# natir/br

Hardware: AMD Instinct MI355X
Metric: corrected Gbases/sec at k=19, 10 kb ONT-error reads (higher is better)
Workload: dtype u64 k-mers / 1-bit set

## Files before the change

br_amd/csrc/brx_partbuild.hip:

```cpp
#include "brx_internal.hpp"
#include "brx_index.hpp"

#include <stdlib.h>
#include <string.h>
#include <atomic>

namespace brx {
uint64_t scan_tmp_bytes(uint32_t n);
int exclusive_scan_lens(const uint32_t *d_lens, uint32_t n, uint64_t *d_tmp, uint64_t *d_out_offsets,
                        unsigned long long *d_total, hipStream_t s);
}

using namespace brx;

namespace {

constexpr int F_BITS = 12;
constexpr int MAX_LEVELS = 4;
constexpr int MAX_DIGIT_BITS = 9;
static_assert(MAX_DIGIT_BITS <= 9, "the digit scans of the partition passes are written for at most 512 digits");

struct Plan {
    int k, nbits, nlev;
    int bits[MAX_LEVELS];
// ... 825 lines not shown
                incl += u;
        }
        __syncthreads();
        if ((threadIdx.x & 63) == 63)
            wsum[threadIdx.x >> 6] = incl;
        __syncthreads();
        uint64_t base = poff[p];
        for (uint32_t w = 0; w < (threadIdx.x >> 6); w++)
            base += wsum[w];
        uint64_t run[2];
        run[0] = base + incl - mine;
        run[1] = run[0] + tot[0];
        for (uint32_t q = 0; q < BPT; q++) {
            const uint32_t b = threadIdx.x * BPT + q;
            if (b < B)
                coff[p * B + b] = run[q];
        }
        for (uint64_t t = 0; t < nt; t++)
            for (uint32_t q = 0; q < BPT; q++) {
                const uint32_t b = threadIdx.x * BPT + q;
                if (b < B) {
                    pos[B * (io + t) + b] = run[q];
                    run[q] += m[B * (io + t) + b];
                }
            }
        if (p == n_parents - 1 && threadIdx.x == 0)
            coff[n_parents * B] = poff[n_parents];
    }
}

template <int KPT, typename OUT>
__global__ __launch_bounds__(256) void ln_scatter_kernel(LnArgs a)
{
    extern __shared__ __attribute__((aligned(16))) uint8_t lds_raw[];
    __shared__ uint32_t sh_wsum[4];
    const uint32_t T = a.tile;
    const uint32_t B = 1u << a.bits;
    uint32_t *stage_key = (uint32_t *)lds_raw;
    uint16_t *stage_dig = (uint16_t *)(lds_raw + (size_t)T * 4);
    unsigned long long *gbase = (unsigned long long *)(lds_raw + (size_t)T * 6);
    uint32_t *cntv = (uint32_t *)(lds_raw + (size_t)T * 6 + (size_t)B * 8);
    uint32_t *lofs = cntv + B;
    uint32_t *lcur = lofs + B;
    const int shift = a.rem_in - a.bits;
    const uint32_t child_mask = (1u << shift) - 1u;
    OUT *out = (OUT *)a.keys_out;
    const unsigned long long n_items = *a.n_items;
    const ItemRange ir = xcd_items(n_items);
    if (ir.first >= ir.end)
        return;
    constexpr uint32_t OWN = ((1u << MAX_DIGIT_BITS) + 255u) / 256u;
    auto load_rows = [&](unsigned long long item, uint32_t(&rc)[OWN], uint64_t(&rp)[OWN]) {
#pragma unroll
        for (uint32_t q = 0; q < OWN; q++) {
            const uint32_t b = threadIdx.x + 256u * q;
            const uint64_t mi = B * item + (b < B ? b : 0u);
            rc[q] = a.matrix[mi];
            rp[q] = a.pos[mi];
        }
    };
    LnItem it = ln_item_get(ln_item_load(a, ir.first));
    uint32_t key[KPT], rc[OWN];
    uint64_t rp[OWN];
    load_rows(ir.first, rc, rp);
    ln_load<KPT>(a, it, key);
    for (unsigned long long item = ir.first; item < ir.end; item += ir.step) {
#pragma unroll
        for (uint32_t q = 0; q < OWN; q++) {
            const uint32_t b = threadIdx.x + 256u * q;
            if (b < B) {
                cntv[b] = rc[q];
                gbase[b] = rp[q];
            }
        }
        const uint32_t cnt = ln_count(it);
        __syncthreads();
        block_scan_bins(B, cntv, lofs, lcur, sh_wsum);
        __syncthreads();
#pragma unroll
        for (int q = 0; q < KPT; q++)
            if ((uint32_t)q < cnt) {
                const uint32_t d = (key[q] >> shift) & (B - 1u);
                const uint32_t slot = atomicAdd(&lcur[d], 1u);
                stage_key[slot] = key[q] & child_mask;
                stage_dig[slot] = (uint16_t)d;
            }
        __syncthreads();
        const uint32_t n_tile = lofs[B - 1] + cntv[B - 1];
        for (uint32_t idx = threadIdx.x; idx < n_tile; idx += 256) {
            const uint32_t d = stage_dig[idx];
            const uint64_t at = gbase[d] + (idx - lofs[d]);
            if (store_ok(at, a.out_cap))
                out[at] = (OUT)stage_key[idx];
        }
        const unsigned long long next = item + ir.step;
        if (next < ir.end) {
            it = ln_item_get(ln_item_load(a, next));
            load_rows(next, rc, rp);
            ln_load<KPT>(a, it, key);
        }
        __syncthreads();
    }
}

constexpr int P3_WAVES = 4;
constexpr uint32_t F_SIZE = 1u << F_BITS;
constexpr uint32_t CNT_WORDS = F_SIZE / 2;
constexpr uint32_t BIT_WORDS = F_SIZE / 32;
constexpr uint32_t CHUNK_MAX = 65000;

constexpr uint32_t STAGE_KEYS = 704;

constexpr uint32_t EMIT_CAP = 256;

template <bool EMIT, bool BITS>
__global__ __launch_bounds__(64 * P3_WAVES) void final_count_kernel(const uint16_t *__restrict__ keys,
                                                                     const uint64_t *__restrict__ off, uint64_t n_buckets,
                                                                     uint32_t abundance, uint32_t *__restrict__ bits,
                                                                     uint64_t *__restrict__ emit_keys, uint64_t emit_cap,
                                                                     unsigned long long *__restrict__ emit_n)
{
    __shared__ uint32_t cnt_all[P3_WAVES][CNT_WORDS];
    __shared__ uint32_t bit_all[P3_WAVES][BIT_WORDS];
    __shared__ __attribute__((aligned(8))) uint16_t stage_all[P3_WAVES][STAGE_KEYS + 8];
    __shared__ uint64_t emit_all[EMIT ? P3_WAVES : 1][EMIT ? EMIT_CAP : 1];
    const int wave = threadIdx.x >> 6, lane = threadIdx.x & 63;
    uint32_t *cnt = cnt_all[wave];
    uint32_t *bmp = bit_all[wave];
    uint16_t *stage = stage_all[wave];
    uint64_t *ebuf = emit_all[EMIT ? wave : 0];
    uint32_t ecount = 0;
    auto emit_flush = [&]() {
        if (ecount) {
            unsigned long long base = 0;
            if (lane == 0)
                base = atomicAdd(emit_n, (unsigned long long)ecount);
            base = __shfl(base, 0);
            asm volatile("" ::: "memory");
            for (uint32_t q = lane; q < ecount; q += 64)
                if (base + q < emit_cap)
                    emit_keys[base + q] = ebuf[q];
            asm volatile("" ::: "memory");
            ecount = 0;
        }
    };
    for (uint32_t w = lane; w < CNT_WORDS; w += 64)
        cnt[w] = 0;
    for (uint32_t w = lane; w < BIT_WORDS; w += 64)
        bmp[w] = 0;
    auto emit_if = [&](bool flag, uint64_t hkey) {
        const uint64_t bal = __ballot(flag);
        if (bal) {
            if (ecount + 64u > EMIT_CAP)
                emit_flush();
            if (flag)
                ebuf[ecount + __builtin_amdgcn_mbcnt_hi((uint32_t)(bal >> 32), __builtin_amdgcn_mbcnt_lo((uint32_t)bal, 0u))] = hkey;
            ecount += (uint32_t)__builtin_popcountll(bal);
        }
    };
    asm volatile("" ::: "memory");

    const uint64_t n_waves = (uint64_t)gridDim.x * P3_WAVES;
    const uint64_t wid = (uint64_t)blockIdx.x * P3_WAVES + wave;
    const uint64_t per = (n_buckets + n_waves - 1) / n_waves;
    const uint64_t b_lo = wid * per;
    const uint64_t b_hi = (b_lo + per < n_buckets) ? b_lo + per : n_buckets;

    uint64_t g0 = b_lo;
    while (g0 < b_hi) {
        int gmax = (int)((b_hi - g0 < 63) ? b_hi - g0 : 63);
        const uint64_t oi = g0 + (uint64_t)lane;
        const uint64_t offv = off[oi <= n_buckets ? oi : n_buckets];
        const uint64_t gs = __shfl(offv, 0);
        const bool fits = lane >= 1 && lane <= gmax && (offv - gs) <= (uint64_t)STAGE_KEYS;
        const uint64_t fm = __ballot(fits) >> 1;
        int gcount = (fm == ~0ull >> 1) ? 63 : __builtin_ctzll(~fm);
        if (gcount > gmax)
            gcount = gmax;
        const bool staged = gcount > 0;
        if (!staged)
            gcount = 1;
        const uint64_t ge = __shfl(offv, gcount);
        const uint64_t base4 = gs & ~3ull;
        if (staged) {
            const uint32_t nquads = (uint32_t)((ge - base4 + 3) / 4);
            const uint2 *src = reinterpret_cast<const uint2 *>(keys + base4);
            uint2 *dstq = reinterpret_cast<uint2 *>(stage);
            for (uint32_t q = lane; q < nquads; q += 64)
                dstq[q] = src[q];
            asm volatile("" ::: "memory");
        }
        const uint32_t off_lo = (uint32_t)offv, off_hi = (uint32_t)(offv >> 32);
        for (int j = 0; j < gcount; j++) {
            const uint64_t s = ((uint64_t)(uint32_t)__builtin_amdgcn_readlane(off_hi, j) << 32) |
                               (uint64_t)(uint32_t)__builtin_amdgcn_readlane(off_lo, j);
            const uint64_t e = ((uint64_t)(uint32_t)__builtin_amdgcn_readlane(off_hi, j + 1) << 32) |
                               (uint64_t)(uint32_t)__builtin_amdgcn_readlane(off_lo, j + 1);
            const uint64_t n = e - s;
            bool any_bit = false;
            if (n == 0) {
            } else if (staged && n <= 64) {
                const bool act = (uint64_t)lane < n;
                const uint32_t key = act ? stage[(uint32_t)(s - base4) + lane] : 0u;
                const uint32_t word = key & (CNT_WORDS - 1u), half = key >> (F_BITS - 1);
                bool hot = false, cross = false;
                if (act) {
                    const uint32_t old = (atomicAdd(&cnt[word], 1u << (16u * half)) >> (16u * half)) & 0xffffu;
                    const uint32_t c = old + 1u;
                    hot = (c > 255u ? 255u : c) > abundance;
                    cross = old == abundance && abundance < 255u;
                    if (BITS && hot)
                        atomicOr(&bmp[key >> 5], 1u << (key & 31u));
                }
                if (BITS)
                    any_bit = __ballot(hot) != 0ull;
                else if (EMIT)
                    emit_if(cross, (g0 + (uint64_t)j) * F_SIZE + (uint64_t)key);
                asm volatile("" ::: "memory");
                if (act)
                    cnt[word] = 0;
            } else {
                any_bit = true;
                uint64_t done = 0;
                while (done < n) {
                    const uint64_t m = (n - done < CHUNK_MAX) ? n - done : CHUNK_MAX;
                    for (uint64_t i = lane; i < m; i += 64) {
                        const uint32_t kk = staged ? (uint32_t)stage[(uint32_t)(s - base4 + done + i)] : (uint32_t)keys[s + done + i];
                        atomicAdd(&cnt[kk & (CNT_WORDS - 1u)], 1u << (16u * (kk >> (F_BITS - 1))));
                    }
                    asm volatile("" ::: "memory");
                    done += m;
                    if (done < n) {
                        for (uint32_t w = lane; w < CNT_WORDS; w += 64) {
                            const uint32_t v = cnt[w];
                            const uint32_t a0 = v & 0xffffu, a1 = v >> 16;
                            cnt[w] = (a0 > 255u ? 255u : a0) | ((a1 > 255u ? 255u : a1) << 16);
                        }
                        asm volatile("" ::: "memory");
                    }
                }
                for (uint32_t w = lane; w < CNT_WORDS; w += 64) {
                    const uint32_t v = cnt[w];
                    const uint32_t c0 = v & 0xffffu, c1 = v >> 16;
                    const bool s0 = (c0 > 255u ? 255u : c0) > abundance, s1 = (c1 > 255u ? 255u : c1) > abundance;
                    if (BITS) {
                        if (s0)
                            atomicOr(&bmp[w >> 5], 1u << (w & 31u));
                        if (s1)
                            atomicOr(&bmp[(w + CNT_WORDS) >> 5], 1u << (w & 31u));
                    } else if (EMIT) {
                        emit_if(s0, (g0 + (uint64_t)j) * F_SIZE + (uint64_t)w);
                        emit_if(s1, (g0 + (uint64_t)j) * F_SIZE + (uint64_t)(w + CNT_WORDS));
                    }
                    if (v)
                        cnt[w] = 0;
                }
            }
            asm volatile("" ::: "memory");
            if (!BITS)
                continue;
            uint32_t *dst = bits + (g0 + (uint64_t)j) * BIT_WORDS;
            uint32_t w0 = 0, w1 = 0;
            if (any_bit) {
                w0 = bmp[2 * lane];
                w1 = bmp[2 * lane + 1];
                bmp[2 * lane] = 0;
                bmp[2 * lane + 1] = 0;
            }
            *reinterpret_cast<uint2 *>(dst + 2 * lane) = make_uint2(w0, w1);
            asm volatile("" ::: "memory");
            if (EMIT && any_bit) {
                uint64_t rem = (uint64_t)w0 | ((uint64_t)w1 << 32);
                const uint64_t hbase = (g0 + (uint64_t)j) * F_SIZE + 64ull * (uint64_t)lane;
                for (;;) {
                    const uint64_t bal = __ballot(rem != 0ull);
                    if (!bal)
                        break;
                    if (ecount + 64u > EMIT_CAP)
                        emit_flush();
                    if (rem) {
                        const uint32_t pos = ecount + __builtin_amdgcn_mbcnt_hi((uint32_t)(bal >> 32),
                                                                                __builtin_amdgcn_mbcnt_lo((uint32_t)bal, 0u));
                        ebuf[pos] = hbase + (uint64_t)__builtin_ctzll(rem);
                        rem &= rem - 1ull;
                    }
                    ecount += (uint32_t)__builtin_popcountll(bal);
                }
            }
        }
        g0 += (uint64_t)gcount;
    }
    if (EMIT)
        emit_flush();
}

#ifndef BRX_HF_FLAT
#define BRX_HF_FLAT 1
#endif
constexpr bool HF_FLAT = BRX_HF_FLAT != 0;
constexpr uint32_t HF_VALID = 0x80000000u;
constexpr int HF_CHUNK = 8;
constexpr uint32_t HF_MAX_TRIES = 192;
__host__ __device__ constexpr uint32_t hf_ebuf(int team) { return team > 64 ? 1024u : 512u; }

template <int TEAM, int BLOCK>
__global__ __launch_bounds__(BLOCK) void hash_final_kernel(const uint32_t *__restrict__ keys, const uint64_t *__restrict__ off,
                                                         uint64_t n_buckets, int R, uint32_t abundance, uint32_t log_t,
                                                         uint64_t *__restrict__ emit_keys, uint64_t emit_cap,
                                                         unsigned long long *__restrict__ emit_n,
                                                         const unsigned long long *__restrict__ dup, uint32_t min_lt, float ratio_forced)
{
    extern __shared__ __attribute__((aligned(16))) uint8_t hf_lds[];
    constexpr int TEAMS = BLOCK / TEAM;
    constexpr uint32_t EB = hf_ebuf(TEAM);
    const uint32_t MIN_LT = min_lt;
    const uint32_t Tmax = 1u << log_t;
    const int team = threadIdx.x / TEAM, tl = threadIdx.x % TEAM;
    uint32_t *tab = (uint32_t *)hf_lds + (size_t)team * Tmax;
    unsigned long long *ebuf = (unsigned long long *)(hf_lds + (size_t)TEAMS * Tmax * 4) + (size_t)team * EB;
    uint32_t *ctl = (uint32_t *)(hf_lds + (size_t)TEAMS * Tmax * 4 + (size_t)TEAMS * EB * 8) + team * 4;
    auto team_sync = [&]() {
        if (TEAM > 64)
            __syncthreads();
        else
            __builtin_amdgcn_fence(__ATOMIC_ACQ_REL, "wavefront");
    };
    auto flush = [&]() {
        team_sync();
        const uint32_t ne = ctl[0] < EB ? ctl[0] : EB;
        __shared__ unsigned long long sh_base[TEAMS];
        if (tl == 0)
            sh_base[team] = ne ? atomicAdd(emit_n, (unsigned long long)ne) : 0ull;
        team_sync();
        const unsigned long long base = sh_base[team];
        for (uint32_t q = tl; q < ne; q += TEAM)
            if (base + q < emit_cap)
                emit_keys[base + q] = ebuf[q];
        team_sync();
        if (tl == 0)
            ctl[0] = 0;
        team_sync();
    };
    if (tl == 0) {
        ctl[0] = 0;
        ctl[1] = 0;
    }
    team_sync();
    float ratio = 1.0f;
    if (dup) {
        const float d = (float)dup[0], t = (float)dup[1];
        if (t > 0.0f)
            ratio = fminf(1.0f, 1.25f * d / t + 0.01f);
    }
    if (ratio_forced > 0.0f)
        ratio = ratio_forced;
    const uint64_t n_teams = (uint64_t)gridDim.x * TEAMS;
    for (uint64_t b = (uint64_t)blockIdx.x * TEAMS + team; b < n_buckets; b += n_teams) {
        const uint64_t s0 = off[b], n = off[b + 1] - s0;
        if (n == 0)
            continue;
        const uint64_t n_eff = (uint64_t)((float)n * ratio) + 1ull;
        uint32_t lp = 0;
        while (lp < (uint32_t)R && (n_eff >> lp) > (uint64_t)(Tmax / 8u * 5u))
            lp++;
        uint32_t lt = log_t;
        if (lp == 0) {
            const uint32_t want = (uint32_t)n_eff * 5u / 2u;
            lt = MIN_LT < log_t ? MIN_LT : log_t;
            while (lt < log_t && (1u << lt) < want)
                lt++;
        }
        uint32_t T = 1u << lt;
        for (uint32_t pass = 0; pass < (1u << lp);) {
            for (uint32_t q = tl * 4u; q < T; q += TEAM * 4u)
                *(uint4 *)(tab + q) = make_uint4(0u, 0u, 0u, 0u);
            team_sync();
            for (uint64_t i0 = 0; i0 < n; i0 += (uint64_t)TEAM * HF_CHUNK) {
              uint32_t kbuf[HF_CHUNK];
#pragma unroll
              for (int c = 0; c < HF_CHUNK; c++) {
                  const uint64_t i = i0 + (uint64_t)c * TEAM + tl;
                  kbuf[c] = i < n ? keys[s0 + i] : 0xffffffffu;
              }
              if constexpr (HF_FLAT && TEAM > 64) {
#pragma unroll
              for (int c = 0; c < HF_CHUNK; c++) {
                const uint32_t key = kbuf[c];
                uint32_t pend = (key != 0xffffffffu && !(lp && (key >> ((uint32_t)R - lp)) != pass)) ? 1u : 0u;
                uint32_t h = (key * 0x9E3779B1u) >> (32u - lt);
                const uint32_t mine = HF_VALID | (key << 11);
                for (uint32_t tries = 0; __any(pend); tries++) {
                    const uint32_t e = tab[h];
                    uint32_t r = e;
                    if (pend & (uint32_t)(e == 0u))
                        r = atomicCAS(&tab[h], 0u, mine | 1u);
                    const uint32_t won = (uint32_t)(e == 0u) & (uint32_t)(r == 0u);
                    const uint32_t same = (uint32_t)((r & 0xfffff800u) == mine);
                    if (pend & same & (uint32_t)((r & 0x400u) == 0u))
                        atomicAdd(&tab[h], 1u);
                    pend &= ~(won | same) & 1u;
                    if (tries >= HF_MAX_TRIES) {
                        if (pend)
                            ctl[1] = 1;
                        pend = 0;
                    }
                    h = (h + 1u) & (T - 1u);
                }
              }
              } else {
#pragma unroll
              for (int c = 0; c < HF_CHUNK; c++) {
                const uint32_t key = kbuf[c];
                if (key == 0xffffffffu || (lp && (key >> ((uint32_t)R - lp)) != pass))
                    continue;
                uint32_t h = (key * 0x9E3779B1u) >> (32u - lt);
                const uint32_t mine = HF_VALID | (key << 11);
                for (uint32_t tries = 0;; tries++) {
                    uint32_t e = tab[h];
                    if (e == 0u) {
                        e = atomicCAS(&tab[h], 0u, mine | 1u);
                        if (e == 0u)
                            break;
                    }
                    if ((e & 0xfffff800u) == mine) {
                        if ((e & 0x7ffu) < 1024u)
                            atomicAdd(&tab[h], 1u);
                        break;
                    }
                    if (tries >= HF_MAX_TRIES) {
                        ctl[1] = 1;
                        break;
                    }
                    h = (h + 1u) & (T - 1u);
                }
              }
              }
            }
            team_sync();
            const uint32_t ovf = ctl[1];
            team_sync();
            if (ovf) {
                if (tl == 0)
                    ctl[1] = 0;
                team_sync();
                if (lt < log_t) {
                    lt = log_t;
                    T = Tmax;
                    continue;
                }
                if (lp + 2u <= (uint32_t)R) {
                    lp += 2u;
                    pass <<= 2;
                    continue;
                }
            }
            for (uint32_t q0 = tl * 4u; q0 < T; q0 += TEAM * 4u) {
                const uint4 e4 = *(const uint4 *)(tab + q0);
                const uint32_t ev[4] = {e4.x, e4.y, e4.z, e4.w};
#pragma unroll
                for (int j = 0; j < 4; j++) {
                    const uint32_t e = ev[j];
                    const uint32_t cnt = e & 0x7ffu;
                    if ((e & HF_VALID) && (cnt > 255u ? 255u : cnt) > abundance) {
                        const unsigned long long hk = (b << R) | (uint64_t)((e >> 11) & 0xfffffu);
                        const uint32_t pos = atomicAdd(&ctl[0], 1u);
                        if (pos < EB) {
                            ebuf[pos] = hk;
                        } else {
                            const unsigned long long gp = atomicAdd(emit_n, 1ull);
                            if (gp < emit_cap)
                                emit_keys[gp] = hk;
                        }
                    }
                }
            }
            team_sync();
            const uint32_t ec = ctl[0];
            team_sync();
            if (ec > EB / 2u)
                flush();
            pass++;
        }
    }
    flush();
}

__global__ __launch_bounds__(1024) void hf_sample_kernel(const uint32_t *__restrict__ keys, const uint64_t *__restrict__ off,
                                                         uint64_t n_buckets, int R, uint32_t log_t, unsigned long long *__restrict__ dup)
{
    extern __shared__ __attribute__((aligned(16))) uint8_t hf_lds[];
    __shared__ uint32_t sh_new;
    uint32_t *tab = (uint32_t *)hf_lds;
    const uint32_t T = 1u << log_t;
    const uint64_t b = (uint64_t)blockIdx.x * n_buckets / gridDim.x;
    const uint64_t s0 = off[b], n = off[b + 1] - s0;
    if (threadIdx.x == 0)
        sh_new = 0;
    uint32_t lp = 0;
    while (lp < (uint32_t)R && (n >> lp) > (uint64_t)(T / 8u * 5u))
        lp++;
    uint32_t fresh = 0;
    for (uint32_t pass = 0; pass < (1u << lp); pass++) {
        __syncthreads();
        for (uint32_t q = threadIdx.x; q < T; q += 1024u)
            tab[q] = 0;
        __syncthreads();
        for (uint64_t i = threadIdx.x; i < n; i += 1024u) {
            const uint32_t key = keys[s0 + i];
            if (lp && (key >> ((uint32_t)R - lp)) != pass)
                continue;
            uint32_t h = (key * 0x9E3779B1u) >> (32u - log_t);
            const uint32_t mine = HF_VALID | (key << 11);
            for (uint32_t tries = 0; tries < T; tries++) {
                uint32_t e = tab[h];
                if (e == 0u) {
                    e = atomicCAS(&tab[h], 0u, mine);
                    if (e == 0u) {
                        fresh++;
                        break;
                    }
                }
                if (e == mine)
                    break;
                h = (h + 1u) & (T - 1u);
            }
        }
    }
    atomicAdd(&sh_new, fresh);
    __syncthreads();
    if (threadIdx.x == 0) {
        atomicAdd(dup, (unsigned long long)sh_new);
        atomicAdd(dup + 1, (unsigned long long)n);
    }
}

constexpr int SP_WAVES = 4;
__global__ __launch_bounds__(64 * SP_WAVES) void final_spectrum_kernel(const uint16_t *__restrict__ keys, const uint64_t *__restrict__ off,
                                                                       uint64_t n_buckets, unsigned long long *__restrict__ hist)
{
    __shared__ uint32_t sp_cnt[SP_WAVES][F_SIZE];
    __shared__ unsigned long long sp_hist[256];
    const int wave = threadIdx.x / 64, lane = threadIdx.x % 64;
    uint32_t *cnt = sp_cnt[wave];
    for (uint32_t q = lane; q < F_SIZE; q += 64)
        cnt[q] = 0;
    for (uint32_t q = threadIdx.x; q < 256; q += 64 * SP_WAVES)
        sp_hist[q] = 0;
    __syncthreads();
    const uint64_t n_waves = (uint64_t)gridDim.x * SP_WAVES;
    for (uint64_t g = (uint64_t)blockIdx.x * SP_WAVES + wave; g < n_buckets; g += n_waves) {
        const uint64_t s0 = off[g], n = off[g + 1] - s0;
        for (uint64_t i = lane; i < n; i += 64)
            atomicAdd(&cnt[keys[s0 + i]], 1u);
        __builtin_amdgcn_fence(__ATOMIC_ACQ_REL, "wavefront");
        for (uint64_t i = lane; i < n; i += 64) {
            const uint32_t c = atomicExch(&cnt[keys[s0 + i]], 0u);
            if (c)
                atomicAdd(&sp_hist[c > 255u ? 255u : c], 1ull);
        }
        __builtin_amdgcn_fence(__ATOMIC_ACQ_REL, "wavefront");
    }
    __syncthreads();
    for (uint32_t q = threadIdx.x; q < 256; q += 64 * SP_WAVES)
        if (sp_hist[q])
            atomicAdd(&hist[q], sp_hist[q]);
}

constexpr int VW_WAVES = 4;
constexpr uint32_t VIEW_PAD = 0xFFFFu;
constexpr uint64_t VW_PER_WAVE = 63ull * 16ull;
__global__ __launch_bounds__(64 * VW_WAVES) void final_view_kernel(uint16_t *keys, const uint64_t *__restrict__ off, uint64_t n_buckets,
                                                                   uint8_t *__restrict__ cnt_out)
{
    __shared__ uint32_t bins_all[VW_WAVES][F_SIZE];
    __shared__ __attribute__((aligned(8))) uint16_t stage_all[VW_WAVES][STAGE_KEYS + 8];
    __shared__ __attribute__((aligned(4))) uint8_t scnt_all[VW_WAVES][STAGE_KEYS + 8];
    __shared__ uint32_t bmp_all[VW_WAVES][BIT_WORDS];
    const int wave = threadIdx.x >> 6, lane = threadIdx.x & 63;
    uint32_t *bins = bins_all[wave];
    uint16_t *stage = stage_all[wave];
    uint8_t *scnt = scnt_all[wave];
    uint32_t *bmp = bmp_all[wave];
    for (uint32_t q = lane; q < F_SIZE; q += 64)
        bins[q] = 0;
    bmp[2 * lane] = 0;
    bmp[2 * lane + 1] = 0;
    asm volatile("" ::: "memory");

    const uint64_t n_chunks = (n_buckets + VW_PER_WAVE * VW_WAVES - 1) / (VW_PER_WAVE * VW_WAVES);
    for (uint64_t chunk = blockIdx.x; chunk < n_chunks; chunk += gridDim.x) {
        const uint64_t b_lo = (chunk * VW_WAVES + (uint64_t)wave) * VW_PER_WAVE;
        const uint64_t b_hi = b_lo + VW_PER_WAVE < n_buckets ? b_lo + VW_PER_WAVE : n_buckets;
        uint64_t g0 = b_lo;
        while (g0 < b_hi) {
            const int gmax = (int)((b_hi - g0 < 63) ? b_hi - g0 : 63);
            const uint64_t oi = g0 + (uint64_t)lane;
            const uint64_t offv = off[oi <= n_buckets ? oi : n_buckets];
            const uint64_t gs = __shfl(offv, 0);
            const bool fits = lane >= 1 && lane <= gmax && (offv - gs) <= (uint64_t)STAGE_KEYS;
            const uint64_t fm = __ballot(fits) >> 1;
            int gcount = (fm == ~0ull >> 1) ? 63 : __builtin_ctzll(~fm);
            if (gcount > gmax)
                gcount = gmax;
            const bool staged = gcount > 0;
            if (!staged)
                gcount = 1;
            const uint64_t ge = __shfl(offv, gcount);
            if (ge == gs) {
                g0 += (uint64_t)gcount;
                continue;
            }
            const uint64_t base4 = gs & ~3ull;
            const uint32_t nquads = (uint32_t)((ge - base4 + 3) / 4);
            if (staged) {
                const uint2 *src = reinterpret_cast<const uint2 *>(keys + base4);
                uint2 *dstq = reinterpret_cast<uint2 *>(stage);
                for (uint32_t q = lane; q < nquads; q += 64)
                    dstq[q] = src[q];
                asm volatile("" ::: "memory");
            }
            const uint32_t off_lo = (uint32_t)offv, off_hi = (uint32_t)(offv >> 32);
            for (int j = 0; j < gcount; j++) {
                const uint64_t s = ((uint64_t)(uint32_t)__builtin_amdgcn_readlane(off_hi, j) << 32) |
                                   (uint64_t)(uint32_t)__builtin_amdgcn_readlane(off_lo, j);
                const uint64_t e = ((uint64_t)(uint32_t)__builtin_amdgcn_readlane(off_hi, j + 1) << 32) |
                                   (uint64_t)(uint32_t)__builtin_amdgcn_readlane(off_lo, j + 1);
                const uint64_t n = e - s;
                if (n == 0)
                    continue;
                const uint32_t sidx = (uint32_t)(s - base4);
                if (staged && n <= 64) {
                    const bool act = (uint64_t)lane < n;
                    const uint32_t key = act ? (uint32_t)stage[sidx + lane] : VIEW_PAD;
                    uint32_t less = 0, mult = 0, distinct = 0;
                    bool lead = false;
                    for (uint64_t rem = __ballot(act); rem; distinct++) {
                        const int i = __builtin_ctzll(rem);
                        const uint32_t ki = (uint32_t)__builtin_amdgcn_readlane((int)key, i);
                        const uint64_t eq = __ballot(act && key == ki);
                        rem &= ~eq;
                        if (ki < key)
                            less++;
                        if (key == ki) {
                            mult = (uint32_t)__builtin_popcountll(eq);
                            lead = lane == i;
                        }
                    }
                    asm volatile("" ::: "memory");
                    if (act && lead) {
                        stage[sidx + less] = (uint16_t)key;
                        scnt[sidx + less] = (uint8_t)(mult > 255u ? 255u : mult);
                    }
                    if (act && (uint32_t)lane >= distinct) {
                        stage[sidx + lane] = (uint16_t)VIEW_PAD;
                        scnt[sidx + lane] = 0;
                    }
                    asm volatile("" ::: "memory");
                    continue;
                }
                for (uint64_t i = lane; i < n; i += 64) {
                    const uint32_t kk = (staged ? (uint32_t)stage[sidx + (uint32_t)i] : (uint32_t)keys[s + i]) & (F_SIZE - 1u);
                    atomicAdd(&bins[kk], 1u);
                    atomicOr(&bmp[kk >> 5], 1u << (kk & 31u));
                }
                __builtin_amdgcn_fence(__ATOMIC_ACQ_REL, "wavefront");
                uint64_t mine = ((uint64_t)bmp[2 * lane + 1] << 32) | (uint64_t)bmp[2 * lane];
                bmp[2 * lane] = 0;
                bmp[2 * lane + 1] = 0;
                const uint32_t nmine = (uint32_t)__builtin_popcountll(mine);
                uint32_t incl = nmine;
                for (int d = 1; d < 64; d <<= 1) {
                    const uint32_t up = (uint32_t)__shfl_up((int)incl, d);
                    if (lane >= d)
                        incl += up;
                }
                const uint32_t pos = (uint32_t)__shfl((int)incl, 63);
                for (uint32_t p = incl - nmine; mine; mine &= mine - 1ull, p++) {
                    const uint32_t h = 64u * (uint32_t)lane + (uint32_t)__builtin_ctzll(mine);
                    const uint32_t v = bins[h];
                    bins[h] = 0;
                    const uint8_t c8 = (uint8_t)(v > 255u ? 255u : v);
                    if (staged) {
                        stage[sidx + p] = (uint16_t)h;
                        scnt[sidx + p] = c8;
                    } else {
                        keys[s + p] = (uint16_t)h;
                        cnt_out[s + p] = c8;
                    }
                }
                for (uint64_t i = (uint64_t)pos + lane; i < n; i += 64) {
                    if (staged) {
                        stage[sidx + (uint32_t)i] = (uint16_t)VIEW_PAD;
                        scnt[sidx + (uint32_t)i] = 0;
                    } else {
                        keys[s + i] = (uint16_t)VIEW_PAD;
                        cnt_out[s + i] = 0;
                    }
                }
                __builtin_amdgcn_fence(__ATOMIC_ACQ_REL, "wavefront");
            }
            if (staged) {
                asm volatile("" ::: "memory");
                for (uint32_t q = lane; q < nquads; q += 64) {
                    const uint64_t at = base4 + 4ull * q;
                    if (at >= gs && at + 4 <= ge) {
                        *reinterpret_cast<uint2 *>(keys + at) = *reinterpret_cast<const uint2 *>(stage + 4u * q);
                        *reinterpret_cast<uint32_t *>(cnt_out + at) = *reinterpret_cast<const uint32_t *>(scnt + 4u * q);
                    } else {
                        for (uint32_t t = 0; t < 4; t++)
                            if (at + t >= gs && at + t < ge) {
                                keys[at + t] = stage[4u * q + t];
                                cnt_out[at + t] = scnt[4u * q + t];
                            }
                    }
                }
                asm volatile("" ::: "memory");
            }
            g0 += (uint64_t)gcount;
        }
    }
}

__global__ __launch_bounds__(256) void merge_segments_kernel(const uint32_t *__restrict__ src,
                                                             const uint64_t *__restrict__ src_off,
                                                             const uint64_t *__restrict__ dst_off,
                                                             const uint64_t *__restrict__ dst_shift, uint32_t B1,
                                                             uint32_t *__restrict__ dst)
{
    for (uint32_t b = blockIdx.x; b < B1; b += gridDim.x) {
        const uint64_t lo = src_off[b], hi = src_off[b + 1];
        const uint64_t base = dst_off[b] + dst_shift[b];
        for (uint64_t i = lo + threadIdx.x; i < hi; i += blockDim.x)
            dst[base + (i - lo)] = src[i];
    }
}

__global__ void add_counts_kernel(const uint64_t *__restrict__ off, uint32_t B1, uint32_t *__restrict__ counts,
                                  uint64_t *__restrict__ shift_out)
{
    const uint32_t b = blockIdx.x * blockDim.x + threadIdx.x;
    if (b < B1) {
        if (shift_out)
            shift_out[b] = counts[b];
        counts[b] += (uint32_t)(off[b + 1] - off[b]);
    }
}

struct PartBatch {
    uint32_t *d_keys = nullptr;
    uint64_t n = 0;
    uint64_t *d_l1off = nullptr;
    DevBuf<uint32_t> own_keys;
    DevBuf<uint64_t> own_l1off;
    bool borrowed() const { return !own_keys; }
    uint64_t cap() const { return own_keys.cap(); }
};

}

namespace brx {

struct PartState {
    Plan pl;
    Plan pl_wide;
    bool use_wide = false;
    std::vector<PartBatch> batches, spare;
// ... 145 lines not shown
    if (st->batches.empty()) {
        *d_keys = nullptr;
        *d_l1off = nullptr;
        *n_keys = 0;
        return BRX_OK;
    }
    if (st->batches.size() != 1 || st->batches[0].borrowed()) {
        set_error("l1_view needs exactly one locally counted batch (have %zu)", st->batches.size());
        return BRX_ERR_ARG;
    }
    *d_keys = st->batches[0].d_keys;
    *d_l1off = st->batches[0].d_l1off;
    *n_keys = st->batches[0].n;
    return BRX_OK;
}

int part_add_partitioned(brx_counter *c, const uint32_t *d_keys, const uint64_t *d_l1off, uint64_t n_keys)
{
    PartState *st = c->part;
    st->view_valid = false;
    if (n_keys == 0)
        return BRX_OK;
    PartBatch b;
    b.d_keys = const_cast<uint32_t *>(d_keys);
    b.d_l1off = const_cast<uint64_t *>(d_l1off);
    b.n = n_keys;
    st->batches.push_back(std::move(b));
    return BRX_OK;
}

static int ensure_matrix(PartState *st, uint64_t n_entries, uint64_t n_pos)
{
    BRX_TRY(ws_reserve(st->d_matrix, (n_entries + 1) * 4));
    BRX_TRY(ws_reserve(st->d_pos, (n_pos + 2) * 8));
    return ws_reserve(st->d_scan_tmp, scan_tmp_bytes((uint32_t)n_entries) + 64);
}

static size_t scatter_lds_bytes(uint32_t tile, int bits)
{
    const size_t B = (size_t)1 << bits;
    return (size_t)tile * 6 + B * 8 + B * 12 + 64;
}

static size_t l1_scatter_lds_bytes(int bits)
{
    const size_t B = (size_t)1 << bits;
    return (size_t)L1_TILE * 4 + B * 8 + B * 12 + 64;
}

int part_add_batch(brx_counter *c, const uint8_t *d_bases, const uint64_t *d_offsets, uint32_t n_reads,
                   uint64_t total_bases, hipStream_t s)
{
    PartState *st = c->part;
    const Plan &pl = st->pl;
    st->view_valid = false;
    if (total_bases == 0 || n_reads == 0)
        return BRX_OK;
    const uint64_t max_keys = total_bases;
    PartBatch b;
    for (size_t i = 0; i < st->spare.size(); i++)
        if (st->spare[i].cap() >= max_keys) {
            b = std::move(st->spare[i]);
            st->spare.erase(st->spare.begin() + (long)i);
            break;
        }
    if (!b.d_keys) {
        BRX_TRY(ws_reserve(b.own_keys, (max_keys + 1) * 4));
        BRX_TRY(b.own_l1off.reserve(pl.nchild[0] + 1, 0, "partition offsets"));
        b.d_keys = b.own_keys;
        b.d_l1off = b.own_l1off;
    }
    const uint32_t B = 1u << pl.bits[0];
    const uint64_t n_items64 = (total_bases + L1_TILE - 1) / L1_TILE;
    if (n_items64 * B >= (1ull << 32)) {
        set_error("batch of %llu bases is too large for one partition pass; split it", (unsigned long long)total_bases);
        return BRX_ERR_UNSUPPORTED;
    }
    const uint32_t n_items = (uint32_t)n_items64;
    const uint64_t n_entries = (uint64_t)B * n_items;
    const char *genv = getenv("BRX_L1_GRID");
    const long gev = genv ? atol(genv) : 0;
    const uint32_t want_ranges = gev > 0 ? (uint32_t)gev : 2560u;
    const uint32_t n_ranges = n_items < want_ranges ? n_items : want_ranges;
    BRX_TRY(ensure_matrix(st, n_entries, ((uint64_t)n_ranges + 1) * B));
    uint64_t *coltot = st->d_pos + (uint64_t)n_ranges * B;
    L1Args a;
    memset(&a, 0, sizeof(a));
    a.bases = d_bases;
    a.offsets = d_offsets;
    a.n_reads = n_reads;
    a.total = total_bases;
    a.n_items = n_items;
    a.k = pl.k;
    a.nbits = pl.nbits;
    a.bits = pl.bits[0];
    a.matrix = st->d_matrix;
    a.n_ranges = n_ranges;
    a.rsum = st->d_pos;
    a.coff = b.d_l1off;
    a.keys_out = b.d_keys;
    a.out_cap = b.cap();
    {
        KernelTimer t("part_l1_hist", s);
        l1_hist_kernel<<<n_ranges, 256, (size_t)B * 4, s>>>(a);
    }
    trace_stage(s, "partition level 1: histograms");
    {
        KernelTimer t("offsets_scan", s);
        col_scan_columns_kernel<<<B, 256, 0, s>>>(st->d_pos, n_ranges, B, coltot);
        col_scan_digits_kernel<<<1, 64, 0, s>>>(coltot, B, b.d_l1off, st->d_scalars + 1);
    }
    {
        KernelTimer t("part_l1_scatter", s);
        const size_t lds1 = l1_scatter_lds_bytes(a.bits);
        if (lds1 > 64 * 1024)
            BRX_HIP(hipFuncSetAttribute((const void *)l1_scatter_kernel, hipFuncAttributeMaxDynamicSharedMemorySize, (int)lds1));
        l1_scatter_kernel<<<n_ranges, 256, lds1, s>>>(a);
    }
    trace_stage(s, "partition level 1: scatter");
    BRX_HIP(hipGetLastError());
    unsigned long long tot = 0;
    BRX_HIP(hipMemcpyAsync(&tot, st->d_scalars + 1, 8, hipMemcpyDeviceToHost, s));
    BRX_HIP(hipStreamSynchronize(s));
    b.n = tot;
    st->batches.push_back(std::move(b));
    return BRX_OK;
}

template <typename OUT>
static int run_level(PartState *st, int l, const uint32_t *keys_in, const uint64_t *poff, uint64_t n_parents, uint64_t total,
                     void *keys_out, hipStream_t s, const char *tag_hist, const char *tag_scatter)
{
    const Plan &pl = st->use_wide ? st->pl_wide : st->pl;
    const uint32_t B = 1u << pl.bits[l];
    static const bool small_tiles = [] { const char *e = getenv("BRX_SMALL_TILES"); return e && *e == '1'; }();
    const uint32_t tile = (pl.bits[l] > 8 || !small_tiles) ? 8192u : 4096u;
    const uint64_t ub_items = total / tile + n_parents + 1;
    const uint64_t n_entries = (uint64_t)B * ub_items;
    if (n_entries >= (1ull << 32)) {
        set_error("partition level %d needs %llu tile counters; split the input into smaller counters", l + 1,
                  (unsigned long long)n_entries);
        return BRX_ERR_UNSUPPORTED;
    }
    {
        BRX_TRY(ws_reserve(st->d_ntiles, (n_parents + 1) * 4));
        BRX_TRY(ws_reserve(st->d_item_off, (n_parents + 2) * 8));
        BRX_TRY(ws_reserve(st->d_items, (ub_items + 1) * sizeof(LnItem)));
    }
    BRX_TRY(ensure_matrix(st, n_entries > n_parents ? n_entries : n_parents, n_entries > n_parents ? n_entries : n_parents));
    tiles_from_offsets_kernel<<<(unsigned)((n_parents + 255) / 256), 256, 0, s>>>(poff, n_parents, tile, st->d_ntiles);
    BRX_TRY(exclusive_scan_lens(st->d_ntiles, (uint32_t)n_parents, st->d_scan_tmp, st->d_item_off, st->d_scalars, s));
    fill_items_kernel<<<(unsigned)((n_parents + 255) / 256), 256, 0, s>>>(poff, st->d_item_off, n_parents, tile, st->d_items);
    trace_stage(s, tag_hist);
    BRX_HIP(hipMemsetAsync(st->d_matrix, 0, n_entries * 4, s));
    LnArgs a;
    memset(&a, 0, sizeof(a));
    a.keys_in = keys_in;
    a.in_cap = total;
    a.items = st->d_items;
    a.n_items = st->d_scalars;
    a.tile = tile;
    a.rem_in = pl.rem_in[l];
    a.bits = pl.bits[l];
    a.matrix = st->d_matrix;
    a.pos = st->d_pos;
    a.keys_out = keys_out;
    a.out_cap = total + 64;
    const int grid = 256 * 8;
    {
        KernelTimer t(tag_hist, s);
        if (tile == 8192u)
            ln_hist_kernel<32><<<grid, 256, (size_t)B * 4, s>>>(a);
        else
            ln_hist_kernel<16><<<grid, 256, (size_t)B * 4, s>>>(a);
    }
    trace_stage(s, "  histograms done");
    {
        KernelTimer t("offsets_scan", s);
        const unsigned g = n_parents < 4096 ? (unsigned)n_parents : 4096u;
        ln_colscan_kernel<<<g, 256, 0, s>>>(st->d_matrix, poff, st->d_item_off, n_parents, B, st->d_pos, st->d_coff[l]);
    }
    {
        KernelTimer t(tag_scatter, s);
        const size_t lds = scatter_lds_bytes(tile, a.bits);
        if (tile == 8192u)
            ln_scatter_kernel<32, OUT><<<grid, 256, lds, s>>>(a);
        else
            ln_scatter_kernel<16, OUT><<<grid, 256, lds, s>>>(a);
    }
    trace_stage(s, tag_scatter);
    BRX_HIP(hipGetLastError());
    return BRX_OK;
}

static int part_finish_impl(brx_counter *c, uint32_t abundance, hipStream_t s, brx_set *dst, unsigned long long *d_hist,
                            bool view = false)
{
    PartState *st = c->part;
    st->view_valid = false;
    const bool no_set = d_hist || view;
    uint64_t total = 0;
    for (auto &b : st->batches)
        total += b.n;
    const char *e_wide = getenv("BRX_WIDE_L2");
    const uint64_t wide_from = e_wide && *e_wide ? strtoull(e_wide, nullptr, 10) : 16384ull;
    const bool lazy_on = [] { const char *e = getenv("BRX_LAZY_BITS"); return !(e && *e == '0'); }();
    st->use_wide = wide_from != 0 && !no_set && dst && (dst->sparse || (index_wanted(c->k) && lazy_on)) &&
                   st->pl_wide.bits[1] != st->pl.bits[1] &&
                   (wide_from == 1 || (st->pl.nlev == 3 ? total / st->pl.nchild[1] > wide_from
                                                        : total / st->pl_wide.nchild[2] > 640));
    const Plan &pl = st->use_wide ? st->pl_wide : st->pl;
    const uint32_t B1 = (uint32_t)pl.nchild[0];

    const uint32_t *keys1 = nullptr;
    const uint64_t *l1off = nullptr;
    if (st->batches.empty() || total == 0) {
        if (view) {
            st->view_empty = true;
            st->view_valid = true;
        }
        if (no_set)
            return BRX_OK;
        if (dst->sparse) {
            BRX_TRY(dst->d_keylist_n.reserve(1, 0, "key list counter"));
            BRX_HIP(hipMemsetAsync(dst->d_keylist_n, 0, 8, s));
            keylist_mark(dst, true);
        } else {
            BRX_HIP(hipMemsetAsync(dst->d_bits, 0, dst->nwords * 4, s));
            dst->bits_stale = false;
        }
        return BRX_OK;
    } else if (st->batches.size() == 1) {
        keys1 = st->batches[0].d_keys;
        l1off = st->batches[0].d_l1off;
    } else {
        BRX_TRY(ws_reserve(st->d_merged, (total + 1) * 4));
        BRX_TRY(ensure_matrix(st, B1 + 1, B1 + 1));
        BRX_HIP(hipMemsetAsync(st->d_cnts, 0, (uint64_t)B1 * 4, s));
        for (auto &b : st->batches)
            add_counts_kernel<<<(B1 + 255) / 256, 256, 0, s>>>(b.d_l1off, B1, st->d_cnts, nullptr);
        BRX_TRY(exclusive_scan_lens(st->d_cnts, B1, st->d_scan_tmp, st->d_l1off_all, st->d_scalars + 1, s));
        BRX_HIP(hipMemsetAsync(st->d_cnts, 0, (uint64_t)B1 * 4, s));
        for (auto &b : st->batches) {
            add_counts_kernel<<<(B1 + 255) / 256, 256, 0, s>>>(b.d_l1off, B1, st->d_cnts, st->d_shift);
            merge_segments_kernel<<<B1 < 4096u ? B1 : 4096u, 256, 0, s>>>(b.d_keys, b.d_l1off, st->d_l1off_all, st->d_shift, B1,
                                                                         st->d_merged);
        }
        keys1 = st->d_merged;
        l1off = st->d_l1off_all;
    }

    BRX_TRY(ws_reserve(st->d_keys_fin, (total + 64) * 2));
    const bool emit = !no_set && (dst->sparse || index_wanted(c->k));
    const bool lazy = emit && !dst->sparse && lazy_on;
    if (emit) {
        const uint64_t div = (dst->sparse || lazy) ? abundance + 1u : (abundance + 1u > 8u ? abundance + 1u : 8u);
        const uint64_t want = total / div + (1ull << 20);
        BRX_TRY(dst->d_keylist.reserve(want, 0, "solid key list"));
        BRX_TRY(dst->d_keylist_n.reserve(1, 0, "key list counter"));
        BRX_HIP(hipMemsetAsync(dst->d_keylist_n, 0, 8, s));
    }
    static const char *hist_tag[MAX_LEVELS] = {"part_l1_hist", "part_l2_hist", "part_l3_hist", "part_l4_hist"};
    static const char *scat_tag[MAX_LEVELS] = {"part_l1_scatter", "part_l2_scatter", "part_l3_scatter", "part_l4_scatter"};
    if (pl.nlev >= 3)
        BRX_TRY(ws_reserve(st->d_keys_mid, (total + 64) * 4));
    if (pl.nlev >= 4)
        BRX_TRY(ws_reserve(st->d_keys_mid2, (total + 64) * 4));
    const uint32_t *kin = keys1;
    const uint64_t *poff = l1off;
    const bool hf_on = [] { const char *e = getenv("BRX_HASH_FINAL"); return !(e && *e == '0'); }();
    const int R_hf = pl.rem_in[pl.nlev - 1];
    const uint64_t nb_hf = pl.nlev >= 2 ? pl.nchild[pl.nlev - 2] : 0;
    static const uint64_t hf_max_avg = [] { const char *e = getenv("BRX_HASH_FINAL_MAX"); return e && *e ? strtoull(e, nullptr, 10) : 131072ull; }();
    const bool hash_final = !no_set && hf_on && (dst->sparse || lazy) && pl.nlev >= 3 && R_hf <= 20 && total / nb_hf <= hf_max_avg;
    for (int l = 1; l < pl.nlev; l++) {
        if (hash_final && l == pl.nlev - 1)
            break;
        if (l == pl.nlev - 1) {
            BRX_TRY(run_level<uint16_t>(st, l, kin, poff, pl.nchild[l - 1], total, st->d_keys_fin, s, hist_tag[l], scat_tag[l]));
        } else {
            uint32_t *kout = (l & 1) ? st->d_keys_mid : st->d_keys_mid2;
            BRX_TRY(run_level<uint32_t>(st, l, kin, poff, pl.nchild[l - 1], total, kout, s, hist_tag[l], scat_tag[l]));
            kin = kout;
        }
        poff = st->d_coff[l];
    }
    if (hash_final) {
        KernelTimer t("part_hash_final", s);
        const uint64_t avg = total / nb_hf;
        const char *e_logt = getenv("BRX_HF_LOG_T"), *e_minlt = getenv("BRX_HF_MIN_LT"), *e_ratio = getenv("BRX_HF_RATIO");
        const float ratio_forced = e_ratio && *e_ratio ? (float)atof(e_ratio) : 0.0f;
        unsigned long long *dup = st->d_scalars + 2;
        {
            BRX_HIP(hipMemsetAsync(dup, 0, 16, s));
            BRX_HIP(hipFuncSetAttribute((const void *)hf_sample_kernel, hipFuncAttributeMaxDynamicSharedMemorySize, 65536));
            const int ns = (int)(nb_hf < 64ull ? nb_hf : 64ull);
            hf_sample_kernel<<<ns, 1024, 65536, s>>>(kin, poff, nb_hf, R_hf, 14, dup);
        }
        if (avg > 640) {
            uint32_t log_t = 14;
            if (e_logt && *e_logt && atoi(e_logt) >= 6 && atoi(e_logt) <= 14)
                log_t = (uint32_t)atoi(e_logt);
            const uint32_t min_lt = e_minlt && *e_minlt && atoi(e_minlt) >= 4 ? (uint32_t)atoi(e_minlt) : 12u;
            const size_t lds = ((size_t)4 << log_t) + hf_ebuf(1024) * 8 + 16;
            BRX_HIP(hipFuncSetAttribute((const void *)hash_final_kernel<1024, 1024>, hipFuncAttributeMaxDynamicSharedMemorySize, (int)lds));
            const int grid = (int)(nb_hf < 256ull * 4ull ? nb_hf : 256ull * 4ull);
            hash_final_kernel<1024, 1024><<<grid, 1024, lds, s>>>(kin, poff, nb_hf, R_hf, abundance, log_t, dst->d_keylist, dst->d_keylist.cap(),
                                                          dst->d_keylist_n, dup, min_lt, ratio_forced);
        } else {
            uint32_t log_t = 8;
            while (log_t < 11 && (1ull << log_t) < 4 * avg)
                log_t++;
            if (e_logt && *e_logt && atoi(e_logt) >= 6 && atoi(e_logt) <= 11)
                log_t = (uint32_t)atoi(e_logt);
            const uint32_t min_lt = e_minlt && *e_minlt && atoi(e_minlt) >= 4 ? (uint32_t)atoi(e_minlt) : 8u;
            const size_t lds = 4 * (((size_t)4 << log_t) + hf_ebuf(64) * 8 + 16);
            const uint64_t want = (nb_hf + 3) / 4;
            const int grid = (int)(want < 256ull * 16ull ? want : 256ull * 16ull);
            hash_final_kernel<64, 256><<<grid, 256, lds, s>>>(kin, poff, nb_hf, R_hf, abundance, log_t, dst->d_keylist, dst->d_keylist.cap(),
                                                         dst->d_keylist_n, dup, min_lt, ratio_forced);
        }
        BRX_HIP(hipGetLastError());
        trace_stage(s, "hash final");
        keylist_mark(dst, true);
        dst->bits_stale = lazy;
        return BRX_OK;
    }
    const uint64_t *fin_off = st->d_coff[pl.nlev - 1];
    if (view) {
        BRX_TRY(ws_reserve(st->d_view_cnt, total + 64));
        {
            KernelTimer t("part_view", s);
            const uint64_t nb = pl.nchild[pl.nlev - 1];
            const uint64_t chunks = (nb + VW_PER_WAVE * VW_WAVES - 1) / (VW_PER_WAVE * VW_WAVES);
            final_view_kernel<<<read_grid(chunks, 2048u), 64 * VW_WAVES, 0, s>>>(st->d_keys_fin, fin_off, nb, st->d_view_cnt);
        }
        BRX_HIP(hipGetLastError());
        trace_stage(s, "count view");
        BRX_HIP(hipStreamSynchronize(s));
        st->view_empty = false;
        st->view_valid = true;
        return BRX_OK;
    }
    if (d_hist) {
        KernelTimer t("part_spectrum", s);
        const uint64_t nb = pl.nchild[pl.nlev - 1];
        const uint64_t want = (nb + SP_WAVES - 1) / SP_WAVES;
        final_spectrum_kernel<<<(int)(want < 256ull * 8ull ? want : 256ull * 8ull), 64 * SP_WAVES, 0, s>>>(st->d_keys_fin, fin_off, nb, d_hist);
        BRX_HIP(hipGetLastError());
        trace_stage(s, "spectrum");
        return BRX_OK;
    }
    {
        KernelTimer t("part_final_count", s);
        const uint64_t nb = pl.nchild[pl.nlev - 1];
        const uint64_t want_waves = nb < (256ull * 16ull * 8ull) ? nb : (256ull * 16ull * 8ull);
        const int grid = (int)((want_waves + P3_WAVES - 1) / P3_WAVES);
        if (dst->sparse || lazy)
            final_count_kernel<true, false><<<grid, 64 * P3_WAVES, 0, s>>>(st->d_keys_fin, fin_off, nb, abundance, nullptr,
                                                                          dst->d_keylist, dst->d_keylist.cap(), dst->d_keylist_n);
        else if (emit)
            final_count_kernel<true, true><<<grid, 64 * P3_WAVES, 0, s>>>(st->d_keys_fin, fin_off, nb, abundance, dst->d_bits,
                                                                         dst->d_keylist, dst->d_keylist.cap(), dst->d_keylist_n);
        else
            final_count_kernel<false, true><<<grid, 64 * P3_WAVES, 0, s>>>(st->d_keys_fin, fin_off, nb, abundance, dst->d_bits,
                                                                          nullptr, 0, nullptr);
    }
    BRX_HIP(hipGetLastError());
    trace_stage(s, "final count");
    keylist_mark(dst, emit);
    dst->bits_stale = lazy;
    return BRX_OK;
}

int part_finish_into(brx_counter *c, uint32_t abundance, hipStream_t s, brx_set *dst)
{
    const int rc = part_finish_impl(c, abundance, s, dst, nullptr);
#if BRX_DEBUG_BOUNDS
    unsigned long long bad = 0;
    BRX_HIP(hipStreamSynchronize(s));
    BRX_HIP(hipMemcpyFromSymbol(&bad, HIP_SYMBOL(bounds_violations), 8));
    if (bad) {
        set_error("BRX_DEBUG_BOUNDS: %llu scatter stores / key loads of the partition passes were out of range and dropped", bad);
        return BRX_ERR_HIP;
    }
#endif
    return rc;
}

int part_spectrum(brx_counter *c, hipStream_t s, unsigned long long *d_hist)
{
    return part_finish_impl(c, 255u, s, nullptr, d_hist);
}

int part_lookup_prepare(brx_counter *c, hipStream_t s)
{
    if (c->part->view_valid)
        return BRX_OK;
    return part_finish_impl(c, 255u, s, nullptr, nullptr, true);
}

void part_lookup_drop(brx_counter *c)
{
    PartState *st = c->part;
    st->view_valid = false;
    st->d_view_cnt.reset();
}

bool part_lookup_ready(const brx_counter *c) { return c->part && c->part->view_valid; }

bool part_lookup_view(const brx_counter *c, const uint16_t **keys, const uint8_t **counts, const uint64_t **off)
{
    const PartState *st = c->part;
    if (!st || !st->view_valid)
        return false;
    *keys = st->view_empty ? nullptr : st->d_keys_fin.get();
    *counts = st->view_empty ? nullptr : st->d_view_cnt.get();
    *off = st->view_empty ? nullptr : st->d_coff[st->pl.nlev - 1].get();
    return true;
}

bool part_lookup_shape(const brx_counter *c, uint64_t *n_buckets, uint64_t *n_positions)
{
    const PartState *st = c->part;
    if (!st || !st->view_valid)
        return false;
    uint64_t total = 0;
    for (auto &b : st->batches)
        total += b.n;
    *n_buckets = st->pl.nchild[st->pl.nlev - 1];
    *n_positions = st->view_empty ? 0 : total;
    return true;
}

}
```

Before: 27.73.

## Compact linear-probe collisions into per-wave LDS retry queues in hash final

In the 1024-thread hash-final kernel, each key now gets one probe attempt. Keys that collide are compacted into a per-wave LDS queue with their displacement, and the queue is drained in full 64-lane batches. This replaces the earlier loop that kept the whole wave iterating while any lane was still probing. The change also simplifies the threshold test in the emit scan. In exchange it uses extra LDS per block (waves×96×4 bytes) and adds ballot/compaction work and wave barriers on every chunk.

```diff
diff --git a/br_amd/csrc/brx_partbuild.hip b/br_amd/csrc/brx_partbuild.hip
--- a/br_amd/csrc/brx_partbuild.hip
+++ b/br_amd/csrc/brx_partbuild.hip
@@ -1151,6 +1151,36 @@
 constexpr int HF_CHUNK = 8;
 constexpr uint32_t HF_MAX_TRIES = 192;
 __host__ __device__ constexpr uint32_t hf_ebuf(int team) { return team > 64 ? 1024u : 512u; }
+#ifndef BRX_HF_QUEUE
+#define BRX_HF_QUEUE 1
+#endif
+#ifndef BRX_HF_QUEUE_WAVE
+#define BRX_HF_QUEUE_WAVE 0
+#endif
+#ifndef BRX_HF_QCAP
+#define BRX_HF_QCAP 96
+#endif
+#ifndef BRX_HF_SCAN
+#define BRX_HF_SCAN 1
+#endif
+constexpr uint32_t HF_QCAP = BRX_HF_QCAP;
+static_assert(HF_QCAP >= 64u, "a wave pushes up to 64 entries at once");
+static_assert(HF_MAX_TRIES < 256u, "the displacement has 8 bits of a queue entry");
+__host__ __device__ constexpr bool hf_queue(int team) { return team > 64 ? BRX_HF_QUEUE != 0 : BRX_HF_QUEUE_WAVE != 0; }
+__host__ __device__ constexpr size_t hf_qbytes(int team, int block) { return hf_queue(team) ? (size_t)(block / 64) * HF_QCAP * 4 : 0; }
+
+__device__ __forceinline__ bool hf_probe_once(uint32_t *tab, uint32_t h, uint32_t mine, bool act)
+{
+    const uint32_t e = tab[h];
+    uint32_t r = e;
+    if (act & (e == 0u))
+        r = atomicCAS(&tab[h], 0u, mine | 1u);
+    const bool won = (e == 0u) & (r == 0u);
+    const bool same = (r & 0xfffff800u) == mine;
+    if (act & same & ((r & 0x400u) == 0u))
+        atomicAdd(&tab[h], 1u);
+    return act & !(won | same);
+}
 
 template <int TEAM, int BLOCK>
 __global__ __launch_bounds__(BLOCK) void hash_final_kernel(const uint32_t *__restrict__ keys, const uint64_t *__restrict__ off,
@@ -1168,6 +1198,32 @@
     uint32_t *tab = (uint32_t *)hf_lds + (size_t)team * Tmax;
     unsigned long long *ebuf = (unsigned long long *)(hf_lds + (size_t)TEAMS * Tmax * 4) + (size_t)team * EB;
     uint32_t *ctl = (uint32_t *)(hf_lds + (size_t)TEAMS * Tmax * 4 + (size_t)TEAMS * EB * 8) + team * 4;
+    constexpr bool QUEUE = hf_queue(TEAM);
+    uint32_t *const wq = (uint32_t *)(hf_lds + (size_t)TEAMS * Tmax * 4 + (size_t)TEAMS * EB * 8 + (size_t)TEAMS * 16) +
+                         (size_t)(uint32_t)__builtin_amdgcn_readfirstlane((int)(threadIdx.x >> 6)) * HF_QCAP;
+    const uint32_t lane = threadIdx.x & 63u;
+    uint32_t qn = 0, q_lt = 0;
+    auto drain = [&](uint32_t room) {
+        while (qn + room > HF_QCAP) {
+            const uint32_t cnt = qn < 64u ? qn : 64u;
+            const bool act = lane < cnt;
+            qn -= cnt;
+            const uint32_t ent = act ? wq[qn + lane] : 0u;
+            const uint32_t key = ent & 0xfffffu, d = ent >> 20;
+            const uint32_t h = (((key * 0x9E3779B1u) >> (32u - q_lt)) + d) & ((1u << q_lt) - 1u);
+            bool pend = hf_probe_once(tab, h, HF_VALID | (key << 11), act);
+            if (pend && d >= HF_MAX_TRIES) {
+                ctl[1] = 1;
+                pend = false;
+            }
+            const uint64_t bal = __ballot(pend);
+            __builtin_amdgcn_wave_barrier();
+            if (pend)
+                wq[qn + __builtin_amdgcn_mbcnt_hi((uint32_t)(bal >> 32), __builtin_amdgcn_mbcnt_lo((uint32_t)bal, 0u))] = ent + (1u << 20);
+            qn += (uint32_t)__builtin_popcountll(bal);
+            __builtin_amdgcn_wave_barrier();
+        }
+    };
     auto team_sync = [&]() {
         if (TEAM > 64)
             __syncthreads();
@@ -1224,6 +1280,7 @@
             for (uint32_t q = tl * 4u; q < T; q += TEAM * 4u)
                 *(uint4 *)(tab + q) = make_uint4(0u, 0u, 0u, 0u);
             team_sync();
+            q_lt = lt;
             for (uint64_t i0 = 0; i0 < n; i0 += (uint64_t)TEAM * HF_CHUNK) {
               uint32_t kbuf[HF_CHUNK];
 #pragma unroll
@@ -1231,7 +1288,26 @@
                   const uint64_t i = i0 + (uint64_t)c * TEAM + tl;
                   kbuf[c] = i < n ? keys[s0 + i] : 0xffffffffu;
               }
-              if constexpr (HF_FLAT && TEAM > 64) {
+              if constexpr (QUEUE) {
+#pragma unroll
+              for (int c = 0; c < HF_CHUNK; c++) {
+                const uint32_t key = kbuf[c];
+                const bool act = key != 0xffffffffu && !(lp && (key >> ((uint32_t)R - lp)) != pass);
+                if (!__any(act))
+                    continue;
+                const uint32_t h = (key * 0x9E3779B1u) >> (32u - lt);
+                const bool pend = hf_probe_once(tab, h, HF_VALID | (key << 11), act);
+                const uint64_t bal = __ballot(pend);
+                if (bal) {
+                    const uint32_t np = (uint32_t)__builtin_popcountll(bal);
+                    drain(np);
+                    if (pend)
+                        wq[qn + __builtin_amdgcn_mbcnt_hi((uint32_t)(bal >> 32), __builtin_amdgcn_mbcnt_lo((uint32_t)bal, 0u))] = key | (1u << 20);
+                    qn += np;
+                    __builtin_amdgcn_wave_barrier();
+                }
+              }
+              } else if constexpr (HF_FLAT && TEAM > 64) {
 #pragma unroll
               for (int c = 0; c < HF_CHUNK; c++) {
                 const uint32_t key = kbuf[c];
@@ -1285,6 +1361,8 @@
               }
               }
             }
+            if constexpr (QUEUE)
+                drain(HF_QCAP);
             team_sync();
             const uint32_t ovf = ctl[1];
             team_sync();
@@ -1303,6 +1381,7 @@
                     continue;
                 }
             }
+            const uint32_t scan_thr = abundance >= 255u ? 0x7ffu : abundance;
             for (uint32_t q0 = tl * 4u; q0 < T; q0 += TEAM * 4u) {
                 const uint4 e4 = *(const uint4 *)(tab + q0);
                 const uint32_t ev[4] = {e4.x, e4.y, e4.z, e4.w};
@@ -1310,7 +1389,7 @@
                 for (int j = 0; j < 4; j++) {
                     const uint32_t e = ev[j];
                     const uint32_t cnt = e & 0x7ffu;
-                    if ((e & HF_VALID) && (cnt > 255u ? 255u : cnt) > abundance) {
+                    if (BRX_HF_SCAN ? cnt > scan_thr : (e & HF_VALID) && (cnt > 255u ? 255u : cnt) > abundance) {
                         const unsigned long long hk = (b << R) | (uint64_t)((e >> 11) & 0xfffffu);
                         const uint32_t pos = atomicAdd(&ctl[0], 1u);
                         if (pos < EB) {
@@ -2062,7 +2141,7 @@
             if (e_logt && *e_logt && atoi(e_logt) >= 6 && atoi(e_logt) <= 14)
                 log_t = (uint32_t)atoi(e_logt);
             const uint32_t min_lt = e_minlt && *e_minlt && atoi(e_minlt) >= 4 ? (uint32_t)atoi(e_minlt) : 12u;
-            const size_t lds = ((size_t)4 << log_t) + hf_ebuf(1024) * 8 + 16;
+            const size_t lds = ((size_t)4 << log_t) + hf_ebuf(1024) * 8 + 16 + hf_qbytes(1024, 1024);
             BRX_HIP(hipFuncSetAttribute((const void *)hash_final_kernel<1024, 1024>, hipFuncAttributeMaxDynamicSharedMemorySize, (int)lds));
             const int grid = (int)(nb_hf < 256ull * 4ull ? nb_hf : 256ull * 4ull);
             hash_final_kernel<1024, 1024><<<grid, 1024, lds, s>>>(kin, poff, nb_hf, R_hf, abundance, log_t, dst->d_keylist, dst->d_keylist.cap(),
@@ -2074,7 +2153,7 @@
             if (e_logt && *e_logt && atoi(e_logt) >= 6 && atoi(e_logt) <= 11)
                 log_t = (uint32_t)atoi(e_logt);
             const uint32_t min_lt = e_minlt && *e_minlt && atoi(e_minlt) >= 4 ? (uint32_t)atoi(e_minlt) : 8u;
-            const size_t lds = 4 * (((size_t)4 << log_t) + hf_ebuf(64) * 8 + 16);
+            const size_t lds = 4 * (((size_t)4 << log_t) + hf_ebuf(64) * 8 + 16) + hf_qbytes(64, 256);
             const uint64_t want = (nb_hf + 3) / 4;
             const int grid = (int)(want < 256ull * 16ull ? want : 256ull * 16ull);
             hash_final_kernel<64, 256><<<grid, 256, lds, s>>>(kin, poff, nb_hf, R_hf, abundance, log_t, dst->d_keylist, dst->d_keylist.cap(),
```

Measured after the change: 28.16, median of 6. Within noise of the previous version (+1.6%).
